# arkworks-rs/snark

Measured on AMD Instinct MI355X. Metric: R1CS constraints/sec (Groth16 prove, BLS12-381; throughput: 4 proofs in flight per GPU, z resident in HBM), higher is better.
Workload: dtype u32

## Files before the change

### snark_amd/csrc/msm_impl.cuh

```cuda
#pragma once
#include <type_traits>
#include "common.h"

namespace ark355 {

constexpr uint32_t MSM_INVALID = 0xFFFFFFFFu;
#ifdef ARK_DEBUG_SMALL_TABLE
#define ARK_TBL_MASK 0x3FFu
#else
#define ARK_TBL_MASK 0x7FFFFFFFu
#endif
constexpr uint32_t MSM_THREADS = 256;

struct MsmPlan {
  uint64_t n = 0;
  uint32_t c = 0, windows = 0, buckets_per_window = 0, total_buckets = 0;
  uint32_t scalar_bits = 0;
  bool precomp = false;
  uint32_t wstride = 1, table_windows = 0;
  uint32_t key_windows = 0;
  bool negate_high = false;
};

static inline uint32_t msm_seg_len(uint64_t entries, bool pair_lanes, int force = 0) {
// ... 159 lines not shown
      keys[e] = key;
      vals[e] = valid ? ((q * table_stride + i) | ((neg ^ flip) << 31)) : 0u;
    }
    (void)wave_agg_inc(counts, valid ? key : 0u, valid);
    if (++j == wstride) {
      j = 0;
      q++;
    }
  }
}

constexpr uint32_t SCAN_THREADS = 1024;
constexpr uint32_t SCAN_EPT = 16;
static __global__ void __launch_bounds__(SCAN_THREADS)
scan_exclusive_kernel(const uint32_t* __restrict__ in, uint32_t* __restrict__ out, uint32_t m,
                      uint32_t* __restrict__ total, uint32_t span, uint32_t* __restrict__ span_total) {
  __shared__ uint32_t wave_tot[SCAN_THREADS / 64];
  __shared__ uint32_t carry_s;
  const uint32_t tid = threadIdx.x, lane = tid & 63u, wave = tid >> 6;
  if (tid == 0) carry_s = 0;
  __syncthreads();
  constexpr uint32_t TILE = SCAN_THREADS * SCAN_EPT;
  const uint64_t lo = span ? (uint64_t)blockIdx.x * span : 0;
  const uint64_t hi = span ? ((lo + span < m) ? lo + span : (uint64_t)m) : (uint64_t)m;
  for (uint64_t base = lo; base < hi; base += TILE) {
    uint32_t v[SCAN_EPT];
    const uint64_t first = base + (uint64_t)tid * SCAN_EPT;
#pragma unroll
    for (uint32_t q = 0; q < SCAN_EPT / 4; q++) {
      const uint64_t i = first + 4 * q;
      if (i + 3 < m) {
        const uint4 t = *reinterpret_cast<const uint4*>(in + i);
        v[4 * q + 0] = t.x;
        v[4 * q + 1] = t.y;
        v[4 * q + 2] = t.z;
        v[4 * q + 3] = t.w;
      } else {
#pragma unroll
        for (uint32_t k = 0; k < 4; k++) v[4 * q + k] = (i + k < m) ? in[i + k] : 0u;
      }
    }
    uint32_t s = 0;
#pragma unroll
    for (uint32_t k = 0; k < SCAN_EPT; k++) s += v[k];
    uint32_t inc = s;
#pragma unroll
    for (uint32_t d = 1; d < 64; d <<= 1) {
      const uint32_t o = __shfl_up(inc, d, 64);
      if (lane >= d) inc += o;
    }
    if (lane == 63) wave_tot[wave] = inc;
    __syncthreads();
    uint32_t wbase = 0, tile_total = 0;
#pragma unroll
    for (uint32_t w = 0; w < SCAN_THREADS / 64; w++) {
      const uint32_t t = wave_tot[w];
      if (w < wave) wbase += t;
      tile_total += t;
    }
    uint32_t run = carry_s + wbase + (inc - s);
#pragma unroll
    for (uint32_t q = 0; q < SCAN_EPT / 4; q++) {
      const uint64_t i = first + 4 * q;
      uint32_t o[4];
#pragma unroll
      for (uint32_t k = 0; k < 4; k++) {
        o[k] = run;
        run += v[4 * q + k];
      }
      if (i + 3 < m) {
        *reinterpret_cast<uint4*>(out + i) = make_uint4(o[0], o[1], o[2], o[3]);
      } else {
#pragma unroll
        for (uint32_t k = 0; k < 4; k++)
          if (i + k < m) out[i + k] = o[k];
      }
    }
    __syncthreads();
    if (tid == 0) carry_s += tile_total;
    __syncthreads();
  }
  if (tid == 0) {
    if (span) span_total[blockIdx.x] = carry_s;
    else if (total) *total = carry_s;
  }
}
#if defined(ARK_EMUL)
constexpr uint32_t SCAN_SPLIT_MIN = SCAN_THREADS * SCAN_EPT;
#else
constexpr uint32_t SCAN_SPLIT_MIN = 4 * SCAN_THREADS * SCAN_EPT;
#endif
constexpr uint32_t SCAN_MAX_SPANS = 256;
static __global__ void __launch_bounds__(SCAN_THREADS)
scan_add_spans_kernel(uint32_t* __restrict__ out, uint32_t m, uint32_t* __restrict__ total, uint32_t span,
                      const uint32_t* __restrict__ span_total, uint32_t spans) {
  __shared__ uint32_t off_s;
  if (threadIdx.x == 0) {
    uint32_t o = 0;
    for (uint32_t g = 0; g < blockIdx.x; g++) o += span_total[g];
    off_s = o;
    if (blockIdx.x + 1 == spans && total) *total = o + span_total[blockIdx.x];
  }
  __syncthreads();
  const uint32_t off = off_s;
  if (off == 0) return;
  const uint64_t lo = (uint64_t)blockIdx.x * span;
  const uint64_t hi = (lo + span < m) ? lo + span : (uint64_t)m;
  for (uint64_t i = lo + 4ull * threadIdx.x; i < hi; i += 4ull * SCAN_THREADS) {
    if (i + 3 < hi) {
      uint4 t = *reinterpret_cast<uint4*>(out + i);
      t.x += off; t.y += off; t.z += off; t.w += off;
      *reinterpret_cast<uint4*>(out + i) = t;
    } else {
      for (uint64_t k = i; k < hi; k++) out[k] += off;
    }
  }
}
static inline void scan_exclusive(hipStream_t stream, const uint32_t* in, uint32_t* out, uint32_t m, uint32_t* total, DevBuf& aux) {
  constexpr uint32_t TILE = SCAN_THREADS * SCAN_EPT;
  if (m <= SCAN_SPLIT_MIN) {
    ARK_LAUNCH(scan_exclusive_kernel, dim3(1), dim3(SCAN_THREADS), 0, stream, in, out, m, total, 0u, (uint32_t*)nullptr);
    ARK_CHECK_LAUNCH();
    return;
  }
  uint32_t tiles = (m + TILE - 1) / TILE;
  uint32_t tiles_per_span = (tiles + SCAN_MAX_SPANS - 1) / SCAN_MAX_SPANS;
  if (tiles_per_span < 1) tiles_per_span = 1;
  const uint32_t span = tiles_per_span * TILE;
  const uint32_t spans = (m + span - 1) / span;
  aux.ensure((size_t)SCAN_MAX_SPANS * 4);
  ARK_LAUNCH(scan_exclusive_kernel, dim3(spans), dim3(SCAN_THREADS), 0, stream, in, out, m, (uint32_t*)nullptr, span, aux.as<uint32_t>());
  ARK_CHECK_LAUNCH();
  ARK_LAUNCH(scan_add_spans_kernel, dim3(spans), dim3(SCAN_THREADS), 0, stream, out, m, total, span, (const uint32_t*)aux.as<uint32_t>(), spans);
  ARK_CHECK_LAUNCH();
}

static __global__ void __launch_bounds__(MSM_THREADS)
msm_scatter_kernel(const uint32_t* __restrict__ keys, const uint32_t* __restrict__ vals, uint64_t entries,
                   const uint32_t* __restrict__ offsets, uint32_t* __restrict__ cursor,
                   uint32_t* __restrict__ sorted_keys, uint32_t* __restrict__ sorted_vals) {
  const uint64_t e = (uint64_t)blockIdx.x * blockDim.x + threadIdx.x;
  const uint32_t key = (e < entries) ? keys[e] : MSM_INVALID;
  const bool valid = key != MSM_INVALID;
  const uint32_t slot = wave_agg_inc(cursor, valid ? key : 0u, valid);
  if (valid) {
    const uint32_t pos = offsets[key] + slot;
    sorted_keys[pos] = key;
    sorted_vals[pos] = vals[e];
  }
}

constexpr uint32_t SORT_LO_BITS = 8;
constexpr uint32_t SORT_LO = 1u << SORT_LO_BITS;
#ifndef ARK_SORT_MAX_BINS
#define ARK_SORT_MAX_BINS 4096u
#endif
constexpr uint32_t SORT_MAX_BINS = ARK_SORT_MAX_BINS;
constexpr uint32_t SORT_SPT = 4;
constexpr uint32_t SORT_HI_THREADS = 1024;
constexpr uint32_t SORT_EPT = 16;
constexpr uint32_t SORT_TILE = MSM_THREADS * SORT_EPT;

template <class Fr, class Fn>
ARK_D void msm_for_each_digit(Fr k, int mont, uint32_t i, uint32_t n, uint32_t c, uint32_t windows, int precomp_flags,
                              uint32_t table_stride, Fn&& fn) {
  if (mont) k = Fr::from_mont(k);
  const uint32_t wstride = (uint32_t)precomp_flags >> 8;
  const uint32_t flip = ((precomp_flags & MSM_DIGITS_NEGATE_HIGH) && msm_negate_if_high(k)) ? 1u : 0u;
  const uint32_t B = 1u << (c - 1);
  const uint32_t full = 1u << c;
  uint32_t carry = 0;
  uint32_t q = 0, j = 0;
  for (uint32_t w = 0; w < windows; w++) {
    const uint32_t bit = w * c;
    const uint32_t limb = bit >> 5, off = bit & 31;
    uint32_t d = 0;
    if (limb < (uint32_t)Fr::N) {
      uint64_t v = k.l[limb];
      if (limb + 1 < (uint32_t)Fr::N) v |= (uint64_t)k.l[limb + 1] << 32;
      d = (uint32_t)(v >> off) & (full - 1);
    }
    d += carry;
    uint32_t neg = 0;
    if (d > B) {
      d = full - d;
      neg = 1;
      carry = 1;
    } else {
      carry = 0;
    }
    if (d != 0) {
      const uint32_t key = j * B + d - 1;
      const uint32_t val = (q * table_stride + i) | ((neg ^ flip) << 31);
      fn(w, key, val);
    }
    if (++j == wstride) {
      j = 0;
      q++;
    }
  }
}

template <class Fr>
__global__ void __launch_bounds__(SORT_HI_THREADS)
sort_hi_hist_kernel(const Fr* __restrict__ scalars, uint32_t n, int mont, uint32_t c, uint32_t windows, int precomp,
                    uint32_t table_stride, uint32_t bins, uint32_t* __restrict__ hist ) {
  __shared__ uint32_t lds[SORT_MAX_BINS];
  for (uint32_t b = threadIdx.x; b < bins; b += blockDim.x) lds[b] = 0;
  __syncthreads();
  const uint32_t base = blockIdx.x * (SORT_HI_THREADS * SORT_SPT);
  for (uint32_t j = 0; j < SORT_SPT; j++) {
    const uint32_t i = base + j * SORT_HI_THREADS + threadIdx.x;
    if (i < n) {
      msm_for_each_digit<Fr>(scalars[i], mont, i, n, c, windows, precomp, table_stride,
                             [&](uint32_t, uint32_t key, uint32_t) { atomicAdd(&lds[key >> SORT_LO_BITS], 1u); });
    }
  }
  __syncthreads();
  for (uint32_t b = threadIdx.x; b < bins; b += blockDim.x) hist[(size_t)b * gridDim.x + blockIdx.x] = lds[b];
}

template <class Fr>
__global__ void __launch_bounds__(SORT_HI_THREADS)
sort_hi_scatter_kernel(const Fr* __restrict__ scalars, uint32_t n, int mont, uint32_t c, uint32_t windows,
                       int precomp, uint32_t table_stride, uint32_t bins,
                       const uint32_t* __restrict__ hist_scanned ,
                       uint2* __restrict__ tmp ) {
  __shared__ uint32_t lds[SORT_MAX_BINS];
  for (uint32_t b = threadIdx.x; b < bins; b += blockDim.x) lds[b] = hist_scanned[(size_t)b * gridDim.x + blockIdx.x];
  __syncthreads();
  const uint32_t base = blockIdx.x * (SORT_HI_THREADS * SORT_SPT);
  for (uint32_t j = 0; j < SORT_SPT; j++) {
    const uint32_t i = base + j * SORT_HI_THREADS + threadIdx.x;
    if (i < n) {
      msm_for_each_digit<Fr>(scalars[i], mont, i, n, c, windows, precomp, table_stride,
                             [&](uint32_t, uint32_t key, uint32_t val) {
                               const uint32_t pos = atomicAdd(&lds[key >> SORT_LO_BITS], 1u);
                               tmp[pos] = make_uint2(key, val);
                             });
    }
  }
}

template <bool SCATTER>
static __global__ void __launch_bounds__(MSM_THREADS)
sort_lo_kernel(const uint2* __restrict__ tmp ,
               const uint32_t* __restrict__ total_ptr, uint32_t* __restrict__ counts,
               const uint32_t* __restrict__ offsets, uint32_t* __restrict__ cursor,
               uint32_t* __restrict__ sorted_keys, uint32_t* __restrict__ sorted_vals) {
  __shared__ uint32_t cnt[SORT_LO];
  __shared__ uint32_t base_s[SORT_LO];
  const uint32_t total = *total_ptr;
  const uint64_t t0 = (uint64_t)blockIdx.x * SORT_TILE;
  if (t0 >= total) return;
  const uint32_t first = (uint32_t)t0;
  const uint32_t last = (first + SORT_TILE < total) ? first + SORT_TILE : total;
  uint32_t key[SORT_EPT], val[SORT_EPT];
#pragma unroll
  for (uint32_t j = 0; j < SORT_EPT; j++) {
    const uint32_t e = first + j * MSM_THREADS + threadIdx.x;
    if (SCATTER) {
      const uint2 t = (e < last) ? tmp[e] : make_uint2(MSM_INVALID, 0u);
      key[j] = t.x;
      val[j] = t.y;
    } else {
      key[j] = (e < last) ? tmp[e].x : MSM_INVALID;
    }
  }
  const uint32_t h0 = tmp[first].x >> SORT_LO_BITS, h1 = tmp[last - 1].x >> SORT_LO_BITS;
  for (uint32_t hb = h0; hb <= h1; hb++) {
    for (uint32_t t = threadIdx.x; t < SORT_LO; t += blockDim.x) cnt[t] = 0;
    __syncthreads();
#pragma unroll
    for (uint32_t j = 0; j < SORT_EPT; j++) {
      if (key[j] != MSM_INVALID && (key[j] >> SORT_LO_BITS) == hb) atomicAdd(&cnt[key[j] & (SORT_LO - 1)], 1u);
    }
    __syncthreads();
    for (uint32_t t = threadIdx.x; t < SORT_LO; t += blockDim.x) {
      const uint32_t k = (hb << SORT_LO_BITS) | t;
      const uint32_t n_k = cnt[t];
      if (SCATTER) {
        base_s[t] = n_k ? offsets[k] + atomicAdd(&cursor[k], n_k) : 0u;
      } else if (n_k) {
        atomicAdd(&counts[k], n_k);
      }
    }
    if (SCATTER) {
      __syncthreads();
#pragma unroll
      for (uint32_t j = 0; j < SORT_EPT; j++) {
        if (key[j] != MSM_INVALID && (key[j] >> SORT_LO_BITS) == hb) {
          const uint32_t pos = atomicAdd(&base_s[key[j] & (SORT_LO - 1)], 1u);
          sorted_keys[pos] = key[j];
          sorted_vals[pos] = val[j];
        }
      }
    }
    __syncthreads();
  }
}

}
#include "tails28_impl.cuh"
namespace ark355 {

template <class P>
struct is_fp2 {
  static constexpr bool value = false;
};
template <class P>
struct is_fp2<Fp2<P>> {
  static constexpr bool value = true;
};

#ifndef ARK_MSM_HEAVY_SPAN
#define ARK_MSM_HEAVY_SPAN 48
#endif
constexpr uint32_t MSM_HEAVY_SPAN = ARK_MSM_HEAVY_SPAN;
#ifndef ARK_MSM_HEAVY_GRID
#define ARK_MSM_HEAVY_GRID 128u
#endif

template <class F>
ARK_D XYZZ<F> xyzz_shfl_xor(const XYZZ<F>& p, int mask) {
  XYZZ<F> r;
  const uint32_t* src = reinterpret_cast<const uint32_t*>(&p);
  uint32_t* dst = reinterpret_cast<uint32_t*>(&r);
  constexpr int WORDS = sizeof(XYZZ<F>) / 4;
#pragma unroll
  for (int i = 0; i < WORDS; i++) dst[i] = (uint32_t)__shfl_xor((int)src[i], mask, 64);
  return r;
}

template <class F>
ARK_D XYZZ<F> wave_reduce_sum(XYZZ<F> v) {
  for (int mask = 32; mask >= 1; mask >>= 1) {
    XYZZ<F> o = xyzz_shfl_xor(v, mask);
    v = xyzz_add(v, o);
  }
  return v;
}

template <class F>
__global__ void __launch_bounds__(64)
xyzz_sum_kernel(const XYZZ<F>* __restrict__ in, uint32_t count, XYZZ<F>* __restrict__ out) {
  XYZZ<F> v = XYZZ<F>::inf();
  for (uint32_t i = threadIdx.x; i < count; i += 64) v = xyzz_add(v, in[i]);
  v = wave_reduce_sum(v);
  if (threadIdx.x == 0) *out = v;
}

template <class F>
__global__ void __launch_bounds__(MSM_THREADS)
precomp_shift_kernel(const Affine<F>* __restrict__ in, XYZZ<F>* __restrict__ out, uint32_t n, uint32_t c) {
  const uint32_t i = blockIdx.x * blockDim.x + threadIdx.x;
  if (i >= n) return;
  XYZZ<F> p = xyzz_dbl_affine_t<true>(in[i]);
  for (uint32_t k = 1; k < c; k++) p = xyzz_dbl(p);
  out[i] = p;
}

constexpr uint32_t PRE_K = 16;
template <class F>
__global__ void __launch_bounds__(MSM_THREADS)
batch_to_affine_kernel(const XYZZ<F>* __restrict__ in, Affine<F>* __restrict__ out, uint32_t n) {
  const uint32_t t = blockIdx.x * blockDim.x + threadIdx.x;
  const uint64_t first64 = (uint64_t)t * PRE_K;
  if (first64 >= n) return;
  const uint32_t first = (uint32_t)first64;
  const uint32_t cnt = (first + PRE_K <= n) ? PRE_K : (n - first);
  F pref[PRE_K];
  F acc = F::one();
  for (uint32_t j = 0; j < cnt; j++) {
    const XYZZ<F> p = in[first + j];
    if (!p.is_inf()) acc = F::mul_ni(acc, p.zzz);
    pref[j] = acc;
  }
  F inv = F::inv(acc);
  for (uint32_t j = cnt; j-- > 0;) {
    const XYZZ<F> p = in[first + j];
    if (p.is_inf()) {
      out[first + j] = Affine<F>::inf();
      continue;
    }
    const F prev = (j > 0) ? pref[j - 1] : F::one();
    const F i3 = F::mul_ni(inv, prev);
    inv = F::mul_ni(inv, p.zzz);
    const F iz = F::mul_ni(p.zz, i3);
    const F i2 = F::sqr_ni(iz);
    out[first + j] = Affine<F>{F::mul_ni(p.x, i2), F::mul_ni(p.y, i3)};
  }
}

struct PrecompTable {
  MsmPlan plan;
  DevBuf table;
  uint64_t n = 0;
  bool packed = false;
};

template <class F>
static inline size_t table_row_bytes(bool packed) {
  if constexpr (is_fp2<F>::value) {
    using P = typename F::Base::Params;
    return packed ? sizeof(Affine28G2<P, true>) : sizeof(Affine28G2<P, false>);
  } else {
    using P = typename F::Params;
    return packed ? sizeof(Affine28<P>) : sizeof(Affine28U<P>);
  }
}
template <class Fq>
static inline bool table_pack_default(const TunePolicy& pol) {
  if (pol.pack_rows >= 0) return pol.pack_rows != 0;
  return sizeof(Affine28<typename Fq::Params>) % 64 == 0;
}

struct TableNeed {
  uint64_t n;
  uint64_t plan_n;
  bool g2;
  int pref_c = 0;
};

static inline size_t table_budget_bytes(const TunePolicy& pol, size_t scratch_bytes, bool use_free) {
  if (pol.hbm_budget_mb > 0) return (size_t)pol.hbm_budget_mb << 20;
#if defined(ARK_EMUL)
  (void)scratch_bytes;
  (void)use_free;
  return ~(size_t)0 >> 1;
#else
  size_t free_b = 0, total_b = 0;
  if (hipMemGetInfo(&free_b, &total_b) != hipSuccess || total_b == 0) return ~(size_t)0 >> 1;
  size_t budget = total_b / 5 * 4;
  if (use_free && free_b < budget) budget = free_b;
  return budget > scratch_bytes ? budget - scratch_bytes : 0;
#endif
}

template <class Fq, class Fq2, class Fr>
static inline uint32_t table_stride_plan(const TunePolicy& pol, const TableNeed* need, int count, size_t budget, std::string* why,
                                         bool* packed_out = nullptr) {
  bool pk = table_pack_default<Fq>(pol);
  if (packed_out) *packed_out = pk;
  if (pol.table_stride >= 1 && pol.table_stride <= 64) return (uint32_t)pol.table_stride;
  uint32_t max_windows = 1;
// ... 4 lines not shown
      s = 1;
    }
    size_t resident = 0, stage = 0;
    for (int i = 0; i < count; i++) {
      const int pc = need[i].pref_c ? need[i].pref_c : pol.msm_c;
      const MsmPlan p = msm_plan(need[i].n, Fr::Params::BITS, true,
                                 need[i].plan_n ? (int)msm_plan(need[i].plan_n, Fr::Params::BITS, true, 0, 0, pc).c : 0, s, pc);
      if (p.windows > max_windows) max_windows = p.windows;
      const size_t row = need[i].g2 ? table_row_bytes<Fq2>(pk) : table_row_bytes<Fq>(pk);
      const size_t aff = need[i].g2 ? sizeof(Affine<Fq2>) : sizeof(Affine<Fq>);
      const size_t xyzz = need[i].g2 ? sizeof(XYZZ<Fq2>) : sizeof(XYZZ<Fq>);
      resident += (size_t)p.table_windows * need[i].n * row;
      const size_t st = need[i].n * (2 * aff + xyzz);
      if (st > stage) stage = st;
    }
    if (resident + stage <= budget) return s;
    if (s >= max_windows) {
      if (why)
        *why = "window tables do not fit HBM: " + std::to_string((resident + stage) >> 20) + " MiB needed even with one table window, budget " +
               std::to_string(budget >> 20) + " MiB";
      return 0;
    }
  }
}

template <class F>
static void rows_to28(const Affine<F>* src, void* dst, uint64_t n, bool pack, hipStream_t stream) {
  const dim3 grid((uint32_t)((n + 255) / 256));
  if constexpr (is_fp2<F>::value) {
    using P = typename F::Base::Params;
    if (pack)
      ARK_LAUNCH((table_to28_g2_kernel<P, true>), grid, dim3(256), 0, stream, src, static_cast<Affine28G2<P, true>*>(dst), n);
    else
      ARK_LAUNCH((table_to28_g2_kernel<P, false>), grid, dim3(256), 0, stream, src, static_cast<Affine28G2<P, false>*>(dst), n);
  } else {
    using P = typename F::Params;
    if (pack) ARK_LAUNCH((table_to28_kernel<P, true>), grid, dim3(256), 0, stream, src, static_cast<Affine28<P>*>(dst), n);
    else ARK_LAUNCH((table_to28_kernel<P, false>), grid, dim3(256), 0, stream, src, static_cast<Affine28U<P>*>(dst), n);
  }
  ARK_CHECK_LAUNCH();
}

template <class F, class Fr>
static void precomp_build(const TunePolicy& pol, PrecompTable& t, const void* d_bases, uint64_t n, hipStream_t stream,
                          uint64_t plan_n = 0, uint32_t wstride = 1, int pref_c = 0, int packed = -1) {
  t.n = n;
  const int pc = pref_c ? pref_c : pol.msm_c;
  t.plan = msm_plan(n, Fr::Params::BITS, true,
                    plan_n ? (int)msm_plan(plan_n, Fr::Params::BITS, true, 0, 0, pc).c : 0, wstride, pc);
  const MsmPlan& p = t.plan;
  const uint32_t TW = p.table_windows;
  ARK_REQUIRE((uint64_t)TW * n < (1ull << 31), ARK355_EINVAL, "window table too large for 31-bit indices");
  if (pol.trace_host)
    fprintf(stderr, "[ark355] window table: %llu bases, c = %u, %u windows (%u table blocks, %u bucket sets)%s\n",
            (unsigned long long)n, p.c, p.windows, TW, p.key_windows, p.negate_high ? ", scalars above (r - 1) / 2 negated" : "");
  const uint32_t grid = (uint32_t)((n + MSM_THREADS - 1) / MSM_THREADS);
  const uint32_t gridb = (uint32_t)(((n + PRE_K - 1) / PRE_K + MSM_THREADS - 1) / MSM_THREADS);
  const uint32_t shift = p.c * p.wstride;
  bool pack;
  if constexpr (is_fp2<F>::value) pack = packed >= 0 ? packed != 0 : table_pack_default<typename F::Base>(pol);
  else pack = packed >= 0 ? packed != 0 : table_pack_default<F>(pol);
  const size_t row = table_row_bytes<F>(pack);
  t.table.alloc((size_t)TW * (n ? n : 1) * row);
  t.packed = pack;
  if (n == 0) return;
  DevBuf stage[2] = {DevBuf(n * sizeof(Affine<F>)), DevBuf(n * sizeof(Affine<F>))};
  DevBuf tmp(n * sizeof(XYZZ<F>));
  auto encode = [&](const DevBuf& src, uint32_t w) {
    rows_to28<F>(src.as<Affine<F>>(), t.table.as<uint8_t>() + (size_t)w * n * row, n, pack, stream);
  };
  ARK_CHECK_HIP(hipMemcpyAsync(stage[0].p, d_bases, n * sizeof(Affine<F>), hipMemcpyDeviceToDevice, stream));
  encode(stage[0], 0);
  for (uint32_t w = 1; w < TW; w++) {
    DevBuf& prev = stage[(w - 1) & 1];
    DevBuf& cur = stage[w & 1];
    ARK_LAUNCH((precomp_shift_kernel<F>), dim3(grid), dim3(MSM_THREADS), 0, stream, (const Affine<F>*)prev.as<Affine<F>>(),
               tmp.as<XYZZ<F>>(), (uint32_t)n, shift);
    ARK_CHECK_LAUNCH();
    ARK_LAUNCH((batch_to_affine_kernel<F>), dim3(gridb), dim3(MSM_THREADS), 0, stream, (const XYZZ<F>*)tmp.as<XYZZ<F>>(),
               cur.as<Affine<F>>(), (uint32_t)n);
    ARK_CHECK_LAUNCH();
    encode(cur, w);
  }
  ARK_CHECK_HIP(hipStreamSynchronize(stream));
}

struct FillRange {
  void* p;
  uint32_t n16;
  uint32_t rem;
  uint32_t value;
  uint32_t pad;
};
constexpr uint32_t FILL_MAX = 28;
struct FillList {
  FillRange r[FILL_MAX];
  uint32_t count;
};
static __global__ void __launch_bounds__(256) multi_fill_kernel(FillList L) {
  const uint64_t stride = (uint64_t)gridDim.x * blockDim.x;
  for (uint32_t k = 0; k < L.count; k++) {
    const FillRange r = L.r[k];
    const uint4 v = make_uint4(r.value, r.value, r.value, r.value);
    uint4* d = reinterpret_cast<uint4*>(r.p);
    for (uint64_t i = (uint64_t)blockIdx.x * blockDim.x + threadIdx.x; i < r.n16; i += stride) d[i] = v;
    if (blockIdx.x == 0 && threadIdx.x < r.rem) reinterpret_cast<uint32_t*>(r.p)[4ull * r.n16 + threadIdx.x] = r.value;
  }
}
struct FillBatch {
  FillList list;
  hipStream_t stream;
  explicit FillBatch(hipStream_t st) : stream(st) { list.count = 0; }
  void add(void* p, size_t bytes, uint8_t byte_value) {
    if (bytes == 0) return;
    if ((bytes & 3) || (reinterpret_cast<uintptr_t>(p) & 15) || (bytes >> 4) > 0xFFFFFFFFull) {
      ARK_CHECK_HIP(hipMemsetAsync(p, byte_value, bytes, stream));
      return;
    }
    if (list.count == FILL_MAX) flush();
    FillRange& r = list.r[list.count++];
    r.p = p;
    r.n16 = (uint32_t)(bytes >> 4);
    r.rem = (uint32_t)((bytes & 15) >> 2);
    r.value = 0x01010101u * byte_value;
    r.pad = 0;
  }
  void flush() {
    if (list.count == 0) return;
    uint64_t units = 0;
    for (uint32_t k = 0; k < list.count; k++) units += list.r[k].n16;
#if defined(ARK_EMUL)
    const uint32_t grid = 1;
#else
    uint64_t g = (units + 256ull * 8 - 1) / (256ull * 8);
    const uint32_t grid = (uint32_t)(g < 1 ? 1 : (g > 4096 ? 4096 : g));
#endif
    ARK_LAUNCH(multi_fill_kernel, dim3(grid), dim3(256), 0, stream, list);
    ARK_CHECK_LAUNCH();
    list.count = 0;
  }
};
static inline void fill_bytes(FillBatch* fb, void* p, uint8_t v, size_t bytes, hipStream_t stream) {
  if (fb) fb->add(p, bytes, v);
  else ARK_CHECK_HIP(hipMemsetAsync(p, v, bytes, stream));
}

struct MsmSort {
  MsmPlan plan;
  DevBuf keys, vals, counts, offsets, cursor, sorted_keys, sorted_vals, total, hist, hist_scanned, scan_aux;
};

static inline bool msm_sort_one_pass(const MsmPlan& p) { return (p.total_buckets + SORT_LO - 1) / SORT_LO > SORT_MAX_BINS; }

template <class Fr>
static void msm_sort_plan(ark355_ctx* ctx, MsmSort& s, uint64_t n, hipStream_t stream, const PrecompTable* tab = nullptr,
                          FillBatch* fb = nullptr) {
  (void)ctx;
  ARK_REQUIRE(n < (1ull << 31), ARK355_EINVAL, "MSM size must be < 2^31");
  const bool precomp = tab != nullptr;
  if (tab) ARK_REQUIRE(n <= tab->n, ARK355_EINVAL, "more scalars than table rows");
  s.plan = msm_plan(n, Fr::Params::BITS, precomp, tab ? (int)tab->plan.c : 0, tab ? tab->plan.wstride : 0);
  const MsmPlan& p = s.plan;
  const uint64_t entries = (uint64_t)p.windows * n;
  ARK_REQUIRE(entries < (1ull << 31), ARK355_EINVAL, "MSM entry count must be < 2^31");
  const bool two_level = !msm_sort_one_pass(p);
  s.keys.ensure(entries * (two_level ? 8 : 4));
  if (!two_level) s.vals.ensure(entries * 4);
  s.sorted_keys.ensure(entries * 4 + 16);
  s.sorted_vals.ensure(entries * 4 + 16);
  s.counts.ensure((size_t)p.total_buckets * 4);
  s.offsets.ensure((size_t)p.total_buckets * 4);
  s.cursor.ensure((size_t)p.total_buckets * 4);
  s.total.ensure(16);
  if (n == 0) {
    fill_bytes(fb, s.total.p, 0, 4, stream);
    fill_bytes(fb, s.counts.p, 0, (size_t)p.total_buckets * 4, stream);
    fill_bytes(fb, s.offsets.p, 0, (size_t)p.total_buckets * 4, stream);
    return;
  }
  fill_bytes(fb, s.counts.p, 0, (size_t)p.total_buckets * 4, stream);
  fill_bytes(fb, s.cursor.p, 0, (size_t)p.total_buckets * 4, stream);
}

template <class Fr>
static void msm_sort_run(ark355_ctx* ctx, MsmSort& s, const void* d_scalars, uint64_t n, int mont, hipStream_t stream,
                         const PrecompTable* tab = nullptr) {
  const MsmPlan& p = s.plan;
  ARK_REQUIRE(p.n == n, ARK355_EINVAL, "sort was planned for another length");
  if (n == 0) return;
  const uint32_t stride = tab ? (uint32_t)tab->n : 0;
  const uint64_t entries = (uint64_t)p.windows * n;
  const uint32_t bins = (p.total_buckets + SORT_LO - 1) / SORT_LO;
  if (msm_sort_one_pass(p)) {
    const uint32_t grid_n = (uint32_t)((n + MSM_THREADS - 1) / MSM_THREADS);
    ARK_LAUNCH((msm_digits_kernel<Fr>), dim3(grid_n), dim3(MSM_THREADS), 0, stream, (const Fr*)d_scalars, (uint32_t)n,
               mont, p.c, p.windows, msm_digit_flags(p), stride, s.keys.as<uint32_t>(), s.vals.as<uint32_t>(),
               s.counts.as<uint32_t>());
    ARK_CHECK_LAUNCH();
    scan_exclusive(stream, s.counts.as<uint32_t>(), s.offsets.as<uint32_t>(), p.total_buckets, s.total.as<uint32_t>(), s.scan_aux);
    const uint32_t grid_e = (uint32_t)((entries + MSM_THREADS - 1) / MSM_THREADS);
    ARK_LAUNCH(msm_scatter_kernel, dim3(grid_e), dim3(MSM_THREADS), 0, stream, s.keys.as<uint32_t>(),
               s.vals.as<uint32_t>(), entries, s.offsets.as<uint32_t>(), s.cursor.as<uint32_t>(),
               s.sorted_keys.as<uint32_t>(), s.sorted_vals.as<uint32_t>());
    ARK_CHECK_LAUNCH();
    return;
  }
  const uint32_t per_wg = SORT_HI_THREADS * SORT_SPT;
  const uint32_t grid1 = (uint32_t)((n + per_wg - 1) / per_wg);
  const size_t hist_elems = (size_t)bins * grid1;
  s.hist.ensure(hist_elems * 4);
  s.hist_scanned.ensure(hist_elems * 4);
  ARK_LAUNCH((sort_hi_hist_kernel<Fr>), dim3(grid1), dim3(SORT_HI_THREADS), 0, stream, (const Fr*)d_scalars, (uint32_t)n,
             mont, p.c, p.windows, msm_digit_flags(p), stride, bins, s.hist.as<uint32_t>());
  ARK_CHECK_LAUNCH();
  ARK_REQUIRE(hist_elems < (1ull << 31), ARK355_EINVAL, "sort histogram too large");
  scan_exclusive(stream, s.hist.as<uint32_t>(), s.hist_scanned.as<uint32_t>(), (uint32_t)hist_elems, s.total.as<uint32_t>(), s.scan_aux);
  ARK_LAUNCH((sort_hi_scatter_kernel<Fr>), dim3(grid1), dim3(SORT_HI_THREADS), 0, stream, (const Fr*)d_scalars,
             (uint32_t)n, mont, p.c, p.windows, msm_digit_flags(p), stride, bins, s.hist_scanned.as<uint32_t>(),
             s.keys.as<uint2>());
  ARK_CHECK_LAUNCH();
  const uint32_t grid2 = (uint32_t)((entries + SORT_TILE - 1) / SORT_TILE);
  ARK_LAUNCH((sort_lo_kernel<false>), dim3(grid2), dim3(MSM_THREADS), 0, stream, (const uint2*)s.keys.as<uint2>(), s.total.as<uint32_t>(), s.counts.as<uint32_t>(), s.offsets.as<uint32_t>(),
             s.cursor.as<uint32_t>(), s.sorted_keys.as<uint32_t>(), s.sorted_vals.as<uint32_t>());
  ARK_CHECK_LAUNCH();
  scan_exclusive(stream, s.counts.as<uint32_t>(), s.offsets.as<uint32_t>(), p.total_buckets, s.total.as<uint32_t>(), s.scan_aux);
  ARK_LAUNCH((sort_lo_kernel<true>), dim3(grid2), dim3(MSM_THREADS), 0, stream, (const uint2*)s.keys.as<uint2>(), s.total.as<uint32_t>(), s.counts.as<uint32_t>(), s.offsets.as<uint32_t>(),
             s.cursor.as<uint32_t>(), s.sorted_keys.as<uint32_t>(), s.sorted_vals.as<uint32_t>());
  ARK_CHECK_LAUNCH();
}

template <class Fr>
static void msm_sort(ark355_ctx* ctx, MsmSort& s, const void* d_scalars, uint64_t n, int mont, hipStream_t stream,
                     const PrecompTable* tab = nullptr) {
  msm_sort_plan<Fr>(ctx, s, n, stream, tab);
  msm_sort_run<Fr>(ctx, s, d_scalars, n, mont, stream, tab);
}

struct MsmBuckets {
  DevBuf buckets, head, tail, head_key, tail_key, heavy_count, heavy_list;
  DevBuf rc;
  uint32_t seg_len = 32, segs = 0;
  bool prepared = false;
  bool heavy_cleared = false;
};

template <class F>
struct Tail28Of {
  using P = typename F::Params;
  static constexpr bool G2 = false;
};
template <class P_>
struct Tail28Of<Fp2<P_>> {
  using P = P_;
  static constexpr bool G2 = true;
};
template <class F>
static inline size_t msm_slot_bytes() {
  return sizeof(typename Tail28<typename Tail28Of<F>::P, Tail28Of<F>::G2>::Slot);
}
static inline uint32_t msm_parts_count(const MsmPlan& p) { return p.key_windows * p.c; }
template <class F>
static XYZZ<F> msm_parts_finish(const XYZZ<F>* parts, const MsmPlan& p) {
  return msm_finish_host<F>(parts, p.key_windows, p.c);
}

template <class F>
static void msm_prepare_phase(const TunePolicy& pol, const MsmSort& s, MsmBuckets& b, hipStream_t stream, FillBatch* fb = nullptr) {
  const MsmPlan& p = s.plan;
  b.prepared = true;
  b.heavy_cleared = false;
  if (p.n == 0) return;
  const size_t slot = msm_slot_bytes<F>();
  const uint64_t entries = (uint64_t)p.windows * p.n;
  b.seg_len = msm_seg_len(entries, is_fp2<F>::value, pol.msm_seg);
  b.segs = (uint32_t)((entries + b.seg_len - 1) / b.seg_len);
  const uint32_t segs = b.segs;
  b.buckets.ensure((size_t)p.total_buckets * slot);
  b.head.ensure((size_t)segs * slot);
  b.tail.ensure((size_t)segs * slot);
  b.head_key.ensure((size_t)segs * 4);
  b.tail_key.ensure((size_t)segs * 4);
  fill_bytes(fb, b.buckets.p, 0, (size_t)p.total_buckets * slot, stream);
  fill_bytes(fb, b.head_key.p, 0xFF, (size_t)segs * 4, stream);
  fill_bytes(fb, b.tail_key.p, 0xFF, (size_t)segs * 4, stream);
  b.heavy_count.ensure(16);
  fill_bytes(fb, b.heavy_count.p, 0, 4, stream);
  b.heavy_cleared = true;
}

template <class P, int COORDS>
static Msm28Slot<P, COORDS>* msm_slots28(MsmBuckets& b, int which) {
  return (which == 0 ? b.buckets : (which == 1 ? b.head : b.tail)).as<Msm28Slot<P, COORDS>>();
}

template <class F>
static void msm_accumulate_phase(ark355_ctx* ctx, const MsmSort& s, MsmBuckets& b, const void* d_rows, bool packed,
                                 hipStream_t stream, int acc_threads, hipEvent_t ev0 = nullptr, hipEvent_t ev1 = nullptr) {
  const MsmPlan& p = s.plan;
  if (!b.prepared) msm_prepare_phase<F>(ctx->policy, s, b, stream);
  b.prepared = false;
  if (p.n == 0) return;
  const uint32_t segs = b.segs;
  const int acc_want = ctx->policy.acc_threads ? ctx->policy.acc_threads : acc_threads;
  const uint32_t acc_t = (acc_want == 64 || acc_want == 128) ? (uint32_t)acc_want : MSM_THREADS;
  const uint32_t* keys = s.sorted_keys.as<uint32_t>();
  const uint32_t* vals = s.sorted_vals.as<uint32_t>();
  if (ev0) ARK_CHECK_HIP(hipEventRecord(ev0, stream));
  if constexpr (is_fp2<F>::value) {
    using P = typename F::Base::Params;
    if (packed) {
      ARK_LAUNCH((msm_accumulate_g2l28p_kernel<P>), dim3((2 * segs + MSM_THREADS - 1) / MSM_THREADS), dim3(MSM_THREADS), 0, stream,
                 static_cast<const Affine28G2<P, true>*>(d_rows), keys, vals, s.total.as<uint32_t>(), s.offsets.as<uint32_t>(),
                 s.counts.as<uint32_t>(), msm_slots28<P, 8>(b, 0), msm_slots28<P, 8>(b, 1), b.head_key.as<uint32_t>(),
                 msm_slots28<P, 8>(b, 2), b.tail_key.as<uint32_t>(), b.seg_len);
    } else {
      constexpr bool ZL = g2l28_zz_in_lds<P>();
      ARK_LAUNCH((msm_accumulate_g2l28_kernel<P, ZL>), dim3((2 * segs + acc_t - 1) / acc_t), dim3(acc_t),
                 ZL ? ZzLds<P>::bytes(acc_t) : (size_t)0, stream, static_cast<const Affine28G2<P, false>*>(d_rows), keys, vals,
                 s.total.as<uint32_t>(), s.offsets.as<uint32_t>(), s.counts.as<uint32_t>(), msm_slots28<P, 8>(b, 0),
                 msm_slots28<P, 8>(b, 1), b.head_key.as<uint32_t>(), msm_slots28<P, 8>(b, 2), b.tail_key.as<uint32_t>(), b.seg_len);
    }
  } else {
    using P = typename F::Params;
    if (packed) {
      ARK_LAUNCH((msm_accumulate28p_kernel<P>), dim3((segs + MSM_THREADS - 1) / MSM_THREADS), dim3(MSM_THREADS), 0, stream,
                 static_cast<const Affine28<P>*>(d_rows), keys, vals, s.total.as<uint32_t>(), s.offsets.as<uint32_t>(),
                 s.counts.as<uint32_t>(), msm_slots28<P, 4>(b, 0), msm_slots28<P, 4>(b, 1), b.head_key.as<uint32_t>(),
                 msm_slots28<P, 4>(b, 2), b.tail_key.as<uint32_t>(), b.seg_len);
    } else {
      ARK_LAUNCH((msm_accumulate28_kernel<P>), dim3((segs + acc_t - 1) / acc_t), dim3(acc_t), 0, stream,
                 static_cast<const Affine28U<P>*>(d_rows), keys, vals, s.total.as<uint32_t>(), s.offsets.as<uint32_t>(),
                 s.counts.as<uint32_t>(), msm_slots28<P, 4>(b, 0), msm_slots28<P, 4>(b, 1), b.head_key.as<uint32_t>(),
                 msm_slots28<P, 4>(b, 2), b.tail_key.as<uint32_t>(), b.seg_len);
    }
  }
  ARK_CHECK_LAUNCH();
  if (ev1) ARK_CHECK_HIP(hipEventRecord(ev1, stream));
}

template <class F, class Hook = std::nullptr_t>
static bool msm_tails28_launch(ark355_ctx* ctx, int count, const MsmSort* const* sorts, MsmBuckets* const* bks,
                               XYZZ<F>* const* outs, hipStream_t stream, Hook after_merge = nullptr) {
  (void)ctx;
  using P = typename Tail28Of<F>::P;
  constexpr bool G2 = Tail28Of<F>::G2;
  constexpr bool HOOK = !std::is_same<Hook, std::nullptr_t>::value;
  using T = Tail28<P, G2>;
  using Slot = typename T::Slot;
  if (count < 1 || count > TAIL28_MAX) return false;
  const MsmPlan& p0 = sorts[0]->plan;
  const bool empty_with_hook = HOOK && count == 1 && p0.n == 0;
  for (int i = 0; i < count; i++) {
    const MsmPlan& p = sorts[i]->plan;
    if (p.n == 0 && !empty_with_hook) return false;
    if (p.total_buckets != p0.total_buckets || p.buckets_per_window != p0.buckets_per_window || p.key_windows != p0.key_windows ||
        p.c != p0.c)
      return false;
  }
  ARK_REQUIRE(p0.c >= 3 && p0.buckets_per_window == (1u << (p0.c - 1)), ARK355_EINVAL, "bucket layout the 28-bit tails do not know");
  uint32_t lb, hb;
  tails28_split(p0.c, &lb, &hb);
  const uint32_t L = 1u << lb, H = 1u << hb;
  TailBatch28 tb;
  memset(&tb, 0, sizeof(tb));
  uint32_t max_heavy_all = 1;
  for (int i = 0; i < count; i++) {
    const MsmSort& s = *sorts[i];
    MsmBuckets& b = *bks[i];
    const uint32_t segs = b.segs;
    const uint32_t max_heavy = segs / MSM_HEAVY_SPAN + 1;
    const uint32_t avg_span = (uint32_t)(((uint64_t)segs + p0.total_buckets - 1) / p0.total_buckets);
    const uint32_t heavy_span = (2 * avg_span > MSM_HEAVY_SPAN) ? 2 * avg_span : MSM_HEAVY_SPAN;
    if (max_heavy > max_heavy_all) max_heavy_all = max_heavy;
    b.heavy_count.ensure(16);
    b.heavy_list.ensure((size_t)max_heavy * 4);
    b.rc.ensure((size_t)p0.key_windows * (H + L) * sizeof(Slot));
    if (!b.heavy_cleared) ARK_CHECK_HIP(hipMemsetAsync(b.heavy_count.p, 0, 4, stream));
    b.heavy_cleared = false;
    TailJob28& J = tb.j[i];
    J.offsets = s.offsets.as<uint32_t>();
// ... 60 lines not shown
```

### snark_amd/csrc/policy.h

```cpp
#pragma once
#include <stddef.h>
#include <stdint.h>
#include <stdio.h>
#include <stdlib.h>
#include <string.h>

namespace ark355 {

enum Sched : int32_t {
  SCHED_AUTO = -1,
  SCHED_ONE_STREAM = 0,
  SCHED_PIPELINE = 1,
  SCHED_PIPELINE_SYNC = 2,
  SCHED_ONE_STREAM_SPIN = 3,
  SCHED_COUNT = 4
};

struct TunePolicy {
  int32_t sched = SCHED_AUTO;
  int32_t wait_spin = 0;
  int32_t wait_adapt = 0;
  int32_t stream_prio = 1;
  int32_t trace_host = 0;
  int32_t sched_explore = 3;
  int32_t batch_tails = 1;
  int32_t side_g2_tails = 1;
  int32_t side_wm = 1;
  int32_t side_g1_tails = 0;
  int32_t side_h_tails = 1;
  int32_t dwm_loopback = 0;
  int32_t rccl_self = 0;
  int32_t msm_c = 0;
  int32_t msm_c_h = 0;
  int32_t pack_rows = -1;
  int32_t table_stride = 0;
  int64_t hbm_budget_mb = 0;
  int32_t shard_dist_wm = 1;
  int32_t msm_seg = 0;
  int32_t acc_threads = 0;
  int32_t ntt_rmax = 0;
  int32_t ntt_direct_max = -1;
  int32_t ntt_nofuse = 0;
  int32_t check_satisfied = 0;
  int32_t h_eval = -1;
  int32_t pairing_device = -1;
  int32_t pairing_device_min = 256;
  int32_t pairing_each_min = 256;

  struct Field {
    const char* name;
    int kind;
    size_t off;
  };
  static const Field* fields(int* count);

  int set(const char* name, int64_t v);
  int get(const char* name, int64_t* v) const;
  static TunePolicy from_env();
};

#define ARK_POLICY_FIELD32(n, f) {n, 0, offsetof(TunePolicy, f)}
#define ARK_POLICY_FIELD64(n, f) {n, 1, offsetof(TunePolicy, f)}

inline const TunePolicy::Field* TunePolicy::fields(int* count) {
  static const Field tab[] = {
      ARK_POLICY_FIELD32("SCHED", sched),
      ARK_POLICY_FIELD32("WAIT_SPIN", wait_spin),
      ARK_POLICY_FIELD32("WAIT_ADAPT", wait_adapt),
      ARK_POLICY_FIELD32("STREAM_PRIO", stream_prio),
      ARK_POLICY_FIELD32("TRACE_HOST", trace_host),
      ARK_POLICY_FIELD32("SCHED_EXPLORE", sched_explore),
      ARK_POLICY_FIELD32("BATCH_TAILS", batch_tails),
      ARK_POLICY_FIELD32("SIDE_G2_TAILS", side_g2_tails),
      ARK_POLICY_FIELD32("SIDE_WM", side_wm),
      ARK_POLICY_FIELD32("SIDE_H_TAILS", side_h_tails),
      ARK_POLICY_FIELD32("SIDE_G1_TAILS", side_g1_tails),
      ARK_POLICY_FIELD32("MSM_C", msm_c),
      ARK_POLICY_FIELD32("MSM_C_H", msm_c_h),
      ARK_POLICY_FIELD32("PACK_ROWS", pack_rows),
      ARK_POLICY_FIELD32("TABLE_STRIDE", table_stride),
      ARK_POLICY_FIELD64("HBM_BUDGET_MB", hbm_budget_mb),
      ARK_POLICY_FIELD32("SHARD_DIST_WM", shard_dist_wm),
      ARK_POLICY_FIELD32("DWM_LOOPBACK", dwm_loopback),
      ARK_POLICY_FIELD32("RCCL_SELF", rccl_self),
      ARK_POLICY_FIELD32("MSM_SEG", msm_seg),
      ARK_POLICY_FIELD32("ACC_THREADS", acc_threads),
      ARK_POLICY_FIELD32("NTT_RMAX", ntt_rmax),
      ARK_POLICY_FIELD32("NTT_DIRECT_MAX", ntt_direct_max),
      ARK_POLICY_FIELD32("CHECK_SATISFIED", check_satisfied),
      ARK_POLICY_FIELD32("NTT_NOFUSE", ntt_nofuse),
      ARK_POLICY_FIELD32("H_EVAL", h_eval),
      ARK_POLICY_FIELD32("PAIRING_DEVICE", pairing_device),
      ARK_POLICY_FIELD32("PAIRING_DEVICE_MIN", pairing_device_min),
      ARK_POLICY_FIELD32("PAIRING_EACH_MIN", pairing_each_min),
  };
  *count = (int)(sizeof(tab) / sizeof(tab[0]));
  return tab;
}

inline int TunePolicy::set(const char* name, int64_t v) {
  if (!name) return -1;
  if (strcmp(name, "SERIAL") == 0) {
    sched = v < 0 ? SCHED_AUTO : (v ? SCHED_ONE_STREAM : SCHED_PIPELINE);
    return 0;
  }
  if (strcmp(name, "EPILOGUE_SYNC") == 0) {
    if (sched == SCHED_PIPELINE || sched == SCHED_PIPELINE_SYNC) sched = v ? SCHED_PIPELINE_SYNC : SCHED_PIPELINE;
    return 0;
  }
  int n = 0;
  const Field* f = fields(&n);
  for (int i = 0; i < n; i++) {
    if (strcmp(name, f[i].name) != 0) continue;
    char* base = reinterpret_cast<char*>(this) + f[i].off;
    if (f[i].kind == 0) *reinterpret_cast<int32_t*>(base) = (int32_t)v;
    else *reinterpret_cast<int64_t*>(base) = v;
    return 0;
  }
  return -1;
}

inline int TunePolicy::get(const char* name, int64_t* v) const {
  if (!name || !v) return -1;
  int n = 0;
  const Field* f = fields(&n);
  for (int i = 0; i < n; i++) {
    if (strcmp(name, f[i].name) != 0) continue;
    const char* base = reinterpret_cast<const char*>(this) + f[i].off;
    *v = f[i].kind == 0 ? (int64_t)*reinterpret_cast<const int32_t*>(base) : *reinterpret_cast<const int64_t*>(base);
    return 0;
  }
  return -1;
}

inline TunePolicy TunePolicy::from_env() {
  TunePolicy p;
  int n = 0;
  const Field* f = fields(&n);
  char var[64];
  for (int i = 0; i < n; i++) {
    snprintf(var, sizeof(var), "ARK355_%s", f[i].name);
    if (const char* e = getenv(var)) {
      if (e[0]) p.set(f[i].name, strtoll(e, nullptr, 10));
    }
  }
  if (const char* e = getenv("ARK355_SERIAL")) {
    if (e[0]) p.set("SERIAL", e[0] == '1' ? 1 : 0);
  }
  if (const char* e = getenv("ARK355_EPILOGUE_SYNC")) {
    if (e[0]) p.set("EPILOGUE_SYNC", e[0] == '1' ? 1 : 0);
  }
  return p;
}

}
```

Baseline: 51.58 million.

## Stage low-level sort scatter through LDS for coalesced writes, add sort tunables

The second-level bucket sort now ranks each round's entries with LDS atomics, runs a block-wide scan over the per-key counts, and places the entries in LDS in key order. It then writes them to the sorted arrays as contiguous runs instead of scattered per-element global writes. The low-bit width and scalars-per-thread of the high pass also become tunable policy knobs. The staged path is meant to cut uncoalesced global stores, at the cost of extra LDS use, extra barriers, and possibly lower occupancy.

```diff
diff --git a/snark_amd/csrc/msm_impl.cuh b/snark_amd/csrc/msm_impl.cuh
--- a/snark_amd/csrc/msm_impl.cuh
+++ b/snark_amd/csrc/msm_impl.cuh
@@ -335,14 +335,17 @@
 
 constexpr uint32_t SORT_LO_BITS = 8;
 constexpr uint32_t SORT_LO = 1u << SORT_LO_BITS;
+constexpr uint32_t SORT_LO_BITS_MIN = 4;
 #ifndef ARK_SORT_MAX_BINS
 #define ARK_SORT_MAX_BINS 4096u
 #endif
 constexpr uint32_t SORT_MAX_BINS = ARK_SORT_MAX_BINS;
 constexpr uint32_t SORT_SPT = 4;
+constexpr uint32_t SORT_SPT_MAX = 32;
 constexpr uint32_t SORT_HI_THREADS = 1024;
 constexpr uint32_t SORT_EPT = 16;
 constexpr uint32_t SORT_TILE = MSM_THREADS * SORT_EPT;
+static_assert(SORT_LO <= MSM_THREADS, "level 2 scans its key counters with one thread per key");
 
 template <class Fr, class Fn>
 ARK_D void msm_for_each_digit(Fr k, int mont, uint32_t i, uint32_t n, uint32_t c, uint32_t windows, int precomp_flags,
@@ -387,16 +390,17 @@
 template <class Fr>
 __global__ void __launch_bounds__(SORT_HI_THREADS)
 sort_hi_hist_kernel(const Fr* __restrict__ scalars, uint32_t n, int mont, uint32_t c, uint32_t windows, int precomp,
-                    uint32_t table_stride, uint32_t bins, uint32_t* __restrict__ hist ) {
+                    uint32_t table_stride, uint32_t bins, uint32_t lo_bits, uint32_t spt,
+                    uint32_t* __restrict__ hist ) {
   __shared__ uint32_t lds[SORT_MAX_BINS];
   for (uint32_t b = threadIdx.x; b < bins; b += blockDim.x) lds[b] = 0;
   __syncthreads();
-  const uint32_t base = blockIdx.x * (SORT_HI_THREADS * SORT_SPT);
-  for (uint32_t j = 0; j < SORT_SPT; j++) {
+  const uint32_t base = blockIdx.x * (SORT_HI_THREADS * spt);
+  for (uint32_t j = 0; j < spt; j++) {
     const uint32_t i = base + j * SORT_HI_THREADS + threadIdx.x;
     if (i < n) {
       msm_for_each_digit<Fr>(scalars[i], mont, i, n, c, windows, precomp, table_stride,
-                             [&](uint32_t, uint32_t key, uint32_t) { atomicAdd(&lds[key >> SORT_LO_BITS], 1u); });
+                             [&](uint32_t, uint32_t key, uint32_t) { atomicAdd(&lds[key >> lo_bits], 1u); });
     }
   }
   __syncthreads();
@@ -406,33 +410,37 @@
 template <class Fr>
 __global__ void __launch_bounds__(SORT_HI_THREADS)
 sort_hi_scatter_kernel(const Fr* __restrict__ scalars, uint32_t n, int mont, uint32_t c, uint32_t windows,
-                       int precomp, uint32_t table_stride, uint32_t bins,
+                       int precomp, uint32_t table_stride, uint32_t bins, uint32_t lo_bits, uint32_t spt,
                        const uint32_t* __restrict__ hist_scanned ,
                        uint2* __restrict__ tmp ) {
   __shared__ uint32_t lds[SORT_MAX_BINS];
   for (uint32_t b = threadIdx.x; b < bins; b += blockDim.x) lds[b] = hist_scanned[(size_t)b * gridDim.x + blockIdx.x];
   __syncthreads();
-  const uint32_t base = blockIdx.x * (SORT_HI_THREADS * SORT_SPT);
-  for (uint32_t j = 0; j < SORT_SPT; j++) {
+  const uint32_t base = blockIdx.x * (SORT_HI_THREADS * spt);
+  for (uint32_t j = 0; j < spt; j++) {
     const uint32_t i = base + j * SORT_HI_THREADS + threadIdx.x;
     if (i < n) {
       msm_for_each_digit<Fr>(scalars[i], mont, i, n, c, windows, precomp, table_stride,
                              [&](uint32_t, uint32_t key, uint32_t val) {
-                               const uint32_t pos = atomicAdd(&lds[key >> SORT_LO_BITS], 1u);
+                               const uint32_t pos = atomicAdd(&lds[key >> lo_bits], 1u);
                                tmp[pos] = make_uint2(key, val);
                              });
     }
   }
 }
 
-template <bool SCATTER>
+template <bool SCATTER, bool STAGED>
 static __global__ void __launch_bounds__(MSM_THREADS)
 sort_lo_kernel(const uint2* __restrict__ tmp ,
-               const uint32_t* __restrict__ total_ptr, uint32_t* __restrict__ counts,
+               const uint32_t* __restrict__ total_ptr, uint32_t lo_bits, uint32_t* __restrict__ counts,
                const uint32_t* __restrict__ offsets, uint32_t* __restrict__ cursor,
                uint32_t* __restrict__ sorted_keys, uint32_t* __restrict__ sorted_vals) {
   __shared__ uint32_t cnt[SORT_LO];
   __shared__ uint32_t base_s[SORT_LO];
+  __shared__ uint32_t stage_k[STAGED ? SORT_TILE : 1];
+  __shared__ uint32_t stage_v[STAGED ? SORT_TILE : 1];
+  __shared__ uint32_t wave_tot[MSM_THREADS / 64];
+  const uint32_t lo = 1u << lo_bits;
   const uint32_t total = *total_ptr;
   const uint64_t t0 = (uint64_t)blockIdx.x * SORT_TILE;
   if (t0 >= total) return;
@@ -450,17 +458,67 @@
       key[j] = (e < last) ? tmp[e].x : MSM_INVALID;
     }
   }
-  const uint32_t h0 = tmp[first].x >> SORT_LO_BITS, h1 = tmp[last - 1].x >> SORT_LO_BITS;
+  const uint32_t h0 = tmp[first].x >> lo_bits, h1 = tmp[last - 1].x >> lo_bits;
   for (uint32_t hb = h0; hb <= h1; hb++) {
-    for (uint32_t t = threadIdx.x; t < SORT_LO; t += blockDim.x) cnt[t] = 0;
+    for (uint32_t t = threadIdx.x; t < lo; t += blockDim.x) cnt[t] = 0;
     __syncthreads();
+    if (SCATTER && STAGED) {
+      const uint32_t t = threadIdx.x, lane = t & 63u, wave = t >> 6;
+      uint32_t rank[SORT_EPT];
+#pragma unroll
+      for (uint32_t j = 0; j < SORT_EPT; j++) {
+        const bool mine = key[j] != MSM_INVALID && (key[j] >> lo_bits) == hb;
+        rank[j] = mine ? atomicAdd(&cnt[key[j] & (lo - 1)], 1u) : MSM_INVALID;
+      }
+      __syncthreads();
+      const uint32_t n_k = t < lo ? cnt[t] : 0u;
+      uint32_t inc = n_k;
+#pragma unroll
+      for (uint32_t d = 1; d < 64; d <<= 1) {
+        const uint32_t o = __shfl_up(inc, d, 64);
+        if (lane >= d) inc += o;
+      }
+      if (lane == 63) wave_tot[wave] = inc;
+      __syncthreads();
+      uint32_t start = inc - n_k, round_total = 0;
+#pragma unroll
+      for (uint32_t w = 0; w < MSM_THREADS / 64; w++) {
+        const uint32_t wt = wave_tot[w];
+        if (w < wave) start += wt;
+        round_total += wt;
+      }
+      if (t < lo) {
+        const uint32_t k = (hb << lo_bits) | t;
+        const uint32_t g = n_k ? offsets[k] + atomicAdd(&cursor[k], n_k) : 0u;
+        cnt[t] = start;
+        base_s[t] = g - start;
+      }
+      __syncthreads();
+#pragma unroll
+      for (uint32_t j = 0; j < SORT_EPT; j++) {
+        if (rank[j] != MSM_INVALID) {
+          const uint32_t slot = cnt[key[j] & (lo - 1)] + rank[j];
+          stage_k[slot] = key[j];
+          stage_v[slot] = val[j];
+        }
+      }
+      __syncthreads();
+      for (uint32_t s = t; s < round_total; s += MSM_THREADS) {
+        const uint32_t k = stage_k[s];
+        const uint32_t pos = s + base_s[k & (lo - 1)];
+        sorted_keys[pos] = k;
+        sorted_vals[pos] = stage_v[s];
+      }
+      __syncthreads();
+      continue;
+    }
 #pragma unroll
     for (uint32_t j = 0; j < SORT_EPT; j++) {
-      if (key[j] != MSM_INVALID && (key[j] >> SORT_LO_BITS) == hb) atomicAdd(&cnt[key[j] & (SORT_LO - 1)], 1u);
+      if (key[j] != MSM_INVALID && (key[j] >> lo_bits) == hb) atomicAdd(&cnt[key[j] & (lo - 1)], 1u);
     }
     __syncthreads();
-    for (uint32_t t = threadIdx.x; t < SORT_LO; t += blockDim.x) {
-      const uint32_t k = (hb << SORT_LO_BITS) | t;
+    for (uint32_t t = threadIdx.x; t < lo; t += blockDim.x) {
+      const uint32_t k = (hb << lo_bits) | t;
       const uint32_t n_k = cnt[t];
       if (SCATTER) {
         base_s[t] = n_k ? offsets[k] + atomicAdd(&cursor[k], n_k) : 0u;
@@ -472,8 +530,8 @@
       __syncthreads();
 #pragma unroll
       for (uint32_t j = 0; j < SORT_EPT; j++) {
-        if (key[j] != MSM_INVALID && (key[j] >> SORT_LO_BITS) == hb) {
-          const uint32_t pos = atomicAdd(&base_s[key[j] & (SORT_LO - 1)], 1u);
+        if (key[j] != MSM_INVALID && (key[j] >> lo_bits) == hb) {
+          const uint32_t pos = atomicAdd(&base_s[key[j] & (lo - 1)], 1u);
           sorted_keys[pos] = key[j];
           sorted_vals[pos] = val[j];
         }
@@ -784,6 +842,19 @@
 
 static inline bool msm_sort_one_pass(const MsmPlan& p) { return (p.total_buckets + SORT_LO - 1) / SORT_LO > SORT_MAX_BINS; }
 
+struct MsmSortShape {
+  uint32_t lo_bits, spt;
+  bool staged;
+};
+static inline MsmSortShape msm_sort_shape(const TunePolicy& pol, const MsmPlan& p) {
+  MsmSortShape sh;
+  sh.lo_bits = (pol.sort_lo_bits >= (int32_t)SORT_LO_BITS_MIN && pol.sort_lo_bits <= (int32_t)SORT_LO_BITS) ? (uint32_t)pol.sort_lo_bits : SORT_LO_BITS;
+  while (sh.lo_bits < SORT_LO_BITS && ((p.total_buckets + (1u << sh.lo_bits) - 1) >> sh.lo_bits) > SORT_MAX_BINS) sh.lo_bits++;
+  sh.spt = (pol.sort_spt >= 1 && pol.sort_spt <= (int32_t)SORT_SPT_MAX) ? (uint32_t)pol.sort_spt : SORT_SPT;
+  sh.staged = pol.sort_staged != 0;
+  return sh;
+}
+
 template <class Fr>
 static void msm_sort_plan(ark355_ctx* ctx, MsmSort& s, uint64_t n, hipStream_t stream, const PrecompTable* tab = nullptr,
                           FillBatch* fb = nullptr) {
@@ -822,7 +893,6 @@
   if (n == 0) return;
   const uint32_t stride = tab ? (uint32_t)tab->n : 0;
   const uint64_t entries = (uint64_t)p.windows * n;
-  const uint32_t bins = (p.total_buckets + SORT_LO - 1) / SORT_LO;
   if (msm_sort_one_pass(p)) {
     const uint32_t grid_n = (uint32_t)((n + MSM_THREADS - 1) / MSM_THREADS);
     ARK_LAUNCH((msm_digits_kernel<Fr>), dim3(grid_n), dim3(MSM_THREADS), 0, stream, (const Fr*)d_scalars, (uint32_t)n,
@@ -837,27 +907,37 @@
     ARK_CHECK_LAUNCH();
     return;
   }
-  const uint32_t per_wg = SORT_HI_THREADS * SORT_SPT;
+  const MsmSortShape sh = msm_sort_shape(ctx->policy, p);
+  const uint32_t bins = (p.total_buckets + (1u << sh.lo_bits) - 1) >> sh.lo_bits;
+  const uint32_t per_wg = SORT_HI_THREADS * sh.spt;
   const uint32_t grid1 = (uint32_t)((n + per_wg - 1) / per_wg);
   const size_t hist_elems = (size_t)bins * grid1;
   s.hist.ensure(hist_elems * 4);
   s.hist_scanned.ensure(hist_elems * 4);
   ARK_LAUNCH((sort_hi_hist_kernel<Fr>), dim3(grid1), dim3(SORT_HI_THREADS), 0, stream, (const Fr*)d_scalars, (uint32_t)n,
-             mont, p.c, p.windows, msm_digit_flags(p), stride, bins, s.hist.as<uint32_t>());
+             mont, p.c, p.windows, msm_digit_flags(p), stride, bins, sh.lo_bits, sh.spt, s.hist.as<uint32_t>());
   ARK_CHECK_LAUNCH();
   ARK_REQUIRE(hist_elems < (1ull << 31), ARK355_EINVAL, "sort histogram too large");
   scan_exclusive(stream, s.hist.as<uint32_t>(), s.hist_scanned.as<uint32_t>(), (uint32_t)hist_elems, s.total.as<uint32_t>(), s.scan_aux);
   ARK_LAUNCH((sort_hi_scatter_kernel<Fr>), dim3(grid1), dim3(SORT_HI_THREADS), 0, stream, (const Fr*)d_scalars,
-             (uint32_t)n, mont, p.c, p.windows, msm_digit_flags(p), stride, bins, s.hist_scanned.as<uint32_t>(),
-             s.keys.as<uint2>());
+             (uint32_t)n, mont, p.c, p.windows, msm_digit_flags(p), stride, bins, sh.lo_bits, sh.spt,
+             s.hist_scanned.as<uint32_t>(), s.keys.as<uint2>());
   ARK_CHECK_LAUNCH();
   const uint32_t grid2 = (uint32_t)((entries + SORT_TILE - 1) / SORT_TILE);
-  ARK_LAUNCH((sort_lo_kernel<false>), dim3(grid2), dim3(MSM_THREADS), 0, stream, (const uint2*)s.keys.as<uint2>(), s.total.as<uint32_t>(), s.counts.as<uint32_t>(), s.offsets.as<uint32_t>(),
-             s.cursor.as<uint32_t>(), s.sorted_keys.as<uint32_t>(), s.sorted_vals.as<uint32_t>());
+  ARK_LAUNCH((sort_lo_kernel<false, false>), dim3(grid2), dim3(MSM_THREADS), 0, stream, (const uint2*)s.keys.as<uint2>(), s.total.as<uint32_t>(),
+             sh.lo_bits, s.counts.as<uint32_t>(), s.offsets.as<uint32_t>(), s.cursor.as<uint32_t>(), s.sorted_keys.as<uint32_t>(),
+             s.sorted_vals.as<uint32_t>());
   ARK_CHECK_LAUNCH();
   scan_exclusive(stream, s.counts.as<uint32_t>(), s.offsets.as<uint32_t>(), p.total_buckets, s.total.as<uint32_t>(), s.scan_aux);
-  ARK_LAUNCH((sort_lo_kernel<true>), dim3(grid2), dim3(MSM_THREADS), 0, stream, (const uint2*)s.keys.as<uint2>(), s.total.as<uint32_t>(), s.counts.as<uint32_t>(), s.offsets.as<uint32_t>(),
-             s.cursor.as<uint32_t>(), s.sorted_keys.as<uint32_t>(), s.sorted_vals.as<uint32_t>());
+  if (sh.staged) {
+    ARK_LAUNCH((sort_lo_kernel<true, true>), dim3(grid2), dim3(MSM_THREADS), 0, stream, (const uint2*)s.keys.as<uint2>(), s.total.as<uint32_t>(),
+               sh.lo_bits, s.counts.as<uint32_t>(), s.offsets.as<uint32_t>(), s.cursor.as<uint32_t>(), s.sorted_keys.as<uint32_t>(),
+               s.sorted_vals.as<uint32_t>());
+  } else {
+    ARK_LAUNCH((sort_lo_kernel<true, false>), dim3(grid2), dim3(MSM_THREADS), 0, stream, (const uint2*)s.keys.as<uint2>(), s.total.as<uint32_t>(),
+               sh.lo_bits, s.counts.as<uint32_t>(), s.offsets.as<uint32_t>(), s.cursor.as<uint32_t>(), s.sorted_keys.as<uint32_t>(),
+               s.sorted_vals.as<uint32_t>());
+  }
   ARK_CHECK_LAUNCH();
 }
 
diff --git a/snark_amd/csrc/policy.h b/snark_amd/csrc/policy.h
--- a/snark_amd/csrc/policy.h
+++ b/snark_amd/csrc/policy.h
@@ -41,6 +41,9 @@
   int32_t ntt_rmax = 0;
   int32_t ntt_direct_max = -1;
   int32_t ntt_nofuse = 0;
+  int32_t sort_staged = -1;
+  int32_t sort_lo_bits = 0;
+  int32_t sort_spt = 0;
   int32_t check_satisfied = 0;
   int32_t h_eval = -1;
   int32_t pairing_device = -1;
@@ -89,6 +92,9 @@
       ARK_POLICY_FIELD32("NTT_DIRECT_MAX", ntt_direct_max),
       ARK_POLICY_FIELD32("CHECK_SATISFIED", check_satisfied),
       ARK_POLICY_FIELD32("NTT_NOFUSE", ntt_nofuse),
+      ARK_POLICY_FIELD32("SORT_STAGED", sort_staged),
+      ARK_POLICY_FIELD32("SORT_LO_BITS", sort_lo_bits),
+      ARK_POLICY_FIELD32("SORT_SPT", sort_spt),
       ARK_POLICY_FIELD32("H_EVAL", h_eval),
       ARK_POLICY_FIELD32("PAIRING_DEVICE", pairing_device),
       ARK_POLICY_FIELD32("PAIRING_DEVICE_MIN", pairing_device_min),
```

Result: no change. 51.98 million (median of 6 runs) (+0.8%).
